# FanmingL/Recurrent-Offpolicy-RL

Hardware: AMD Instinct MI355X
Metric: env-steps/sec trained (higher is better)
Workload: dtype f32; 1 GPU; smamba_s32_c16_b2_nln SAC-REDQ update, B=64/GPU, T=1024, D=256 (configs[1]; N=8: configs[3]); row_length=1043, obs=17, act=6, critic=efc-8, global_rows=64, parallelism=dp1

## Files before the change

include/resel_hip.h:

```cpp
#ifndef RESEL_HIP_H
#define RESEL_HIP_H

#include <stddef.h>
#include <stdint.h>

#ifdef __cplusplus
extern "C" {
#endif

#define RESEL_OK 0
#define RESEL_EINVAL (-1)
#define RESEL_ELAUNCH (-2)

typedef void* resel_stream_t;

int resel_abi_version(void);
const char* resel_build_info(void);

enum {
    RESEL_PROF_SSCAN_FWD = 0, RESEL_PROF_SSCAN_BWD = 1, RESEL_PROF_ATTN_FWD = 2, RESEL_PROF_ATTN_DQ = 3, RESEL_PROF_ATTN_DKV = 4,
    RESEL_PROF_LINREC_REAL_FWD = 5, RESEL_PROF_LINREC_REAL_BWD = 6, RESEL_PROF_LINREC_COMPLEX_FWD = 7, RESEL_PROF_LINREC_COMPLEX_BWD = 8,
    RESEL_PROF_GRU_FWD = 9, RESEL_PROF_GRU_BWD = 10, RESEL_PROF_CONV_FWD = 11, RESEL_PROF_CONV_BWD = 12, RESEL_PROF_GEMM = 13,
    RESEL_PROF_SSCAN_FWD_LOCAL = 14, RESEL_PROF_SSCAN_BWD_LOCAL = 15,
    RESEL_PROF_NSLOTS = 16
// ... 123 lines not shown
                     const float* seg_lr, const float* seg_wd, int nseg, float beta1, float beta2, float eps,
                     int step, const float* grad_scale, resel_stream_t stream);
int resel_adamw_flat_bc(float* p, const float* g, float* m, float* v, int64_t n, const int64_t* seg_end,
                        const float* seg_lr, const float* seg_wd, int nseg, float beta1, float beta2, float eps,
                        float bc1, float bc2_sqrt, const float* grad_scale, resel_stream_t stream);
int resel_adamw_flat_dev(float* p, const float* g, float* m, float* v, int64_t n, const int64_t* seg_end,
                         const float* seg_lr, const float* seg_wd, int nseg, float beta1, float beta2, float eps,
                         const float* bias_corrections, const float* grad_scale, resel_stream_t stream);
size_t resel_sumsq_workspace_bytes(int64_t n);
int resel_sumsq(const float* x, int64_t n, float* out, void* workspace, resel_stream_t stream);

int resel_bias_act_fwd(float* y, const float* bias, int64_t rows, int C, int64_t rows_per_seg, int act, resel_stream_t stream);
size_t resel_bias_act_bwd_workspace_bytes(int64_t rows, int C, int64_t rows_per_seg);
int resel_bias_act_bwd(const float* g, int64_t ldg, const float* a, int64_t lda, float* gy, float* dbias, void* workspace, int64_t rows, int C,
                       int64_t rows_per_seg, int act, void* amax_gy, unsigned amax_epoch, resel_stream_t stream);

int resel_ensemble_head_fwd(float* y, const float* b2, const float* w3, const float* b3, float* q, int64_t rows, int H,
                            int64_t rows_per_seg, resel_stream_t stream);
size_t resel_ensemble_head_bwd_workspace_bytes(int64_t rows, int H, int64_t rows_per_seg);
int resel_ensemble_head_bwd(const float* gq, const float* a, const float* w3, float* gy, float* db2, float* dw3, void* workspace,
                            int64_t rows, int H, int64_t rows_per_seg, void* amax_gy, unsigned amax_epoch, resel_stream_t stream);

size_t resel_gemm_f32_workspace_bytes(int M, int N, int K, int batch);
int resel_gemm_f32(const float* A, int64_t lda, int64_t strideA, int a_kcontig,
                   const float* B, int64_t ldb, int64_t strideB, int b_kcontig,
                   const float* bias, int64_t strideBias, int act,
                   float* C, int64_t ldc, int64_t strideC, void* workspace,
                   int M, int N, int K, int batch, int split, resel_stream_t stream);

int resel_gemm_f32x(const float* A, int64_t lda, int64_t strideA, int a_kcontig,
// ... 4 lines not shown
                    void* amax_c, unsigned amax_epoch, resel_stream_t stream);
int resel_gemm_f32_fused_supported(int kind, int M, int N, int K, int64_t lda, int64_t ldb);
size_t resel_gemm_f32_fused_workspace_bytes(int M, int N, int K, int batch, int kind);
int resel_gemm_f32_dact(const float* A, int64_t lda, int64_t strideA, int a_kcontig,
                        const float* B, int64_t ldb, int64_t strideB, int b_kcontig,
                        const float* Y, int64_t ldy, int64_t strideY,
                        float* C, int64_t ldc, int64_t strideC, float* dbias, void* workspace,
                        int M, int N, int K, int batch, const float* amax_a, const float* amax_b,
                        void* amax_c, unsigned amax_epoch, resel_stream_t stream);
int resel_gemm_f32_head(const float* A, int64_t lda, int64_t strideA, int a_kcontig,
                        const float* B, int64_t ldb, int64_t strideB, int b_kcontig,
                        const float* bias, int64_t strideBias, const float* w3, int64_t strideW3, const float* b3,
                        float* C, int64_t ldc, int64_t strideC, float* q, void* workspace,
                        int M, int N, int K, int batch, const float* amax_a, const float* amax_b,
                        void* amax_c, unsigned amax_epoch, resel_stream_t stream);
int resel_place_blocks(float* out, int64_t ld_out, int rows, int cols, int nblk, const float* const* src, const int64_t* ld_src,
                       const int* r0, const int* nr, const int* c0, const int* nc, resel_stream_t stream);

int resel_amax_segments(const float* flat, const int64_t* begin, const int64_t* len, int nseg, void* handles, unsigned epoch,
                        resel_stream_t stream);
size_t resel_amax_state_bytes(void);
int resel_amax(const float* x, int64_t ld, int64_t stride, int rows, int cols, int batch, void* out, unsigned epoch, void* state,
               resel_stream_t stream);
int resel_amax_check(const float* x, int64_t ld, int64_t stride, int rows, int cols, int batch, const void* handle, int* err, int tag,
                     resel_stream_t stream);

size_t resel_gemm_bf16_workspace_bytes(int M, int N, int K);
int resel_gemm_bf16(const void* A, int64_t lda, int a_kcontig, int a_bf16, const void* B, int64_t ldb, int b_kcontig, int b_bf16,
                    const float* bias, void* C, int64_t ldc, int c_bf16, void* workspace, int M, int N, int K,
                    resel_stream_t stream);
// ... 28 lines not shown
```

recurrent-offpolicy-rl_amd/csrc/bias_act.hip:

```cpp
#include "resel_common.h"

namespace {
using namespace resel;

constexpr int BWD_ROWS = 128;

__device__ __forceinline__ float elu_(float x) { return x > 0.f ? x : fast_exp(x) - 1.f; }

__global__ __launch_bounds__(256) void bias_act_fwd_kernel(float* __restrict__ y, const float* __restrict__ bias, int64_t rows,
                                                           int C, int64_t rows_per_seg, int act) {
    const int c4n = C / 4;
    const int64_t n4 = rows * c4n;
    for (int64_t i = (int64_t)blockIdx.x * blockDim.x + threadIdx.x; i < n4; i += (int64_t)gridDim.x * blockDim.x) {
        const int64_t r = i / c4n;
        const int c = (int)(i % c4n) * 4;
        float4 v = ld4(y + r * C + c);
        if (bias) {
            const float4 b = ld4(bias + (r / rows_per_seg) * C + c);
            v.x += b.x; v.y += b.y; v.z += b.z; v.w += b.w;
        }
        if (act == 1) { v.x = elu_(v.x); v.y = elu_(v.y); v.z = elu_(v.z); v.w = elu_(v.w); }
        st4(y + r * C + c, v);
    }
}
// ... 87 lines not shown
    amax_publish_wave(gmax, amax);
    st4(&s_red[0][rl][cl * 4], accb);
    st4(&s_red[1][rl][cl * 4], accw);
    __syncthreads();
    if (rl < 2 && c < H) {
        float4 t = ld4(&s_red[rl][0][cl * 4]);
#pragma unroll
        for (int k = 1; k < 4; ++k) {
            const float4 qv = ld4(&s_red[rl][k][cl * 4]);
            t.x += qv.x; t.y += qv.y; t.z += qv.z; t.w += qv.w;
        }
        st4((rl == 0 ? db_part : dw_part) + ((seg * nrb + blockIdx.x) * (int64_t)H) + c, t);
    }
}

inline int row_blocks(int64_t rows_per_seg) { return (int)((rows_per_seg + BWD_ROWS - 1) / BWD_ROWS); }
inline int block_rows(int64_t, int, int64_t) { return BWD_ROWS; }
inline int row_blocks_of(int64_t rows_per_seg, int brows) { return (int)((rows_per_seg + brows - 1) / brows); }
inline bool shape_ok(int64_t rows, int C, int64_t rows_per_seg) {
    return rows > 0 && C > 0 && C % 4 == 0 && rows_per_seg > 0 && rows % rows_per_seg == 0;
}

}

extern "C" int resel_bias_act_fwd(float* y, const float* bias, int64_t rows, int C, int64_t rows_per_seg, int act,
                                  resel_stream_t stream) {
    if (!y || !shape_ok(rows, C, rows_per_seg) || act < 0 || act > 1 || !aligned16(y) || (bias && !aligned16(bias))) return RESEL_EINVAL;
    const int64_t n4 = rows * (C / 4);
    const int64_t want = (n4 + 255) / 256;
    const unsigned grid = (unsigned)(want < 256 * 32 ? want : 256 * 32);
// ... 39 lines not shown
                                       void* workspace, int64_t rows, int H, int64_t rows_per_seg, void* amax_gy, unsigned amax_epoch,
                                       resel_stream_t stream) {
    if (amax_gy && (reinterpret_cast<uintptr_t>(amax_gy) & 7u)) return RESEL_EINVAL;
    if (!gq || !a || !w3 || !gy || !db2 || !dw3 || !workspace || !shape_ok(rows, H, rows_per_seg)) return RESEL_EINVAL;
    if (!aligned16(a) || !aligned16(w3) || !aligned16(gy) || !aligned16(workspace)) return RESEL_EINVAL;
    const int nseg = (int)(rows / rows_per_seg), nrb = row_blocks(rows_per_seg);
    hipStream_t s = (hipStream_t)stream;
    float* db_part = (float*)workspace;
    float* dw_part = db_part + (size_t)nseg * nrb * H;
    hipLaunchKernelGGL(head_bwd_kernel, dim3(nrb, (H + 255) / 256, nseg), dim3(256), 0, s, gq, a, w3, gy, db_part, dw_part, H, rows_per_seg, nrb,
                       AmaxOut{(unsigned long long*)amax_gy, amax_epoch});
    launch_colsum(db_part, H, nrb, H, db2, s, 1, 0, nseg);
    launch_colsum(dw_part, H, nrb, H, dw3, s, 1, 0, nseg);
    return launch_status();
}
```

recurrent-offpolicy-rl_amd/csrc/gemm_bf3.hip:

```cpp
#include "gemm_splitk.h"
#include <type_traits>

namespace {
using namespace resel;

typedef float f32x16 __attribute__((ext_vector_type(16)));
typedef __bf16 bf16x8 __attribute__((ext_vector_type(8)));
constexpr int BM = 256, BN = 128;
constexpr int NTH = 512;
constexpr int GRID = 256;
constexpr int TILE = BM * BN;
constexpr int ROWB = 64;
constexpr int PLA = BM * ROWB, PLB = BN * ROWB;
constexpr int STAGE = 3 * PLA + 3 * PLB;

struct Params {
    const float *A, *B, *bias;
    float *C, *slab;
    int64_t lda, ldb, ldc, sA, sB, sC, sBias;
    int M, N, K;
    int act;
    int mt, nt;
    int nfull, nsplit, nsl, kslice;
    const float *amaxA, *amaxB;
// ... 882 lines not shown
#pragma unroll
                        for (int e = 0; e < 16; ++e) {
                            const int dm = (e & 3) + 8 * (e >> 2);
                            if (mb + dm < p.M) crow[(int64_t)dm * p.ldc] = v[e];
                        }
                    }
                    if (p.amaxC.slot) {
#pragma unroll
                        for (int e = 0; e < 16; e += 2) cmax = fmaxf(cmax, fmaxf(__builtin_fabsf(v[e]), __builtin_fabsf(v[e + 1])));
                    }
                }
            }
        } else {
            float* C = p.C + (int64_t)cur.z * p.sC;
            const bool full_m = cur.m0 + BM <= p.M;
            constexpr bool DACT = EPI == 4, HEAD = EPI == 5;
            const int act = EPI ? (HEAD ? 1 : 0) : p.act;
            if constexpr (DACT) {
                constexpr int PF = 3;
                const int lane = (int)__builtin_amdgcn_mbcnt_hi(~0u, __builtin_amdgcn_mbcnt_lo(~0u, 0u));
                const int li = lane & 31, lh = lane >> 5;
                const int w = __builtin_amdgcn_readfirstlane(threadIdx.x >> 6);
                const int wm = (w >> 1) * 128, wn = (w & 1) * 64;
                typedef float f32x4a __attribute__((ext_vector_type(4)));
                f32x4a yv[8][4];
                char* sc = lds + (w >> 1) * STAGE + 2 * PLA + (w & 1) * 5120;
                float* wr = reinterpret_cast<float*>(sc) + (4 * lh) * 40 + li;
                float4* rdp = reinterpret_cast<float4*>(sc + (lane >> 3) * 160 + (lane & 7) * 16);
                const uint32_t ylane = (uint32_t)(((lane >> 3) * (int)p.ldaux + 4 * (lane & 7)) * 4);
                const float* ybase = p.aux + (int64_t)cur.z * p.sAux + (int64_t)(cur.m0 + wm) * p.ldaux + cur.n0 + wn;
                auto yld = [](f32x4a& r, uint32_t off, const float* base) {
// ... 61 lines not shown
                char* sc = lds + (w >> 1) * STAGE + 2 * PLA + (w & 1) * 5120;
                float* wr = reinterpret_cast<float*>(sc) + (4 * lh) * 40 + li;
                const float4* rdp = reinterpret_cast<const float4*>(sc + (lane >> 3) * 160 + (lane & 7) * 16);
                auto tile = [&](int a, int b, const float4 (&yv)[4], float4& cs, const float4& w3, float (&qr)[4]) {
                    float v[16];
#pragma unroll
                    for (int e = 0; e < 16; ++e) v[e] = acc[a][b][e] + bv[b];
                    if (act == 1) {
#pragma unroll
                        for (int e = 0; e < 16; ++e) v[e] = elu1(v[e]);
                    }
                    if (act == 3) {
#pragma unroll
                        for (int e = 0; e < 16; ++e) v[e] = softplus_nb(v[e]);
                    }
                    if (p.amaxC.slot && !DACT) {
#pragma unroll
                        for (int e = 0; e < 16; e += 2) cmax = fmaxf(cmax, fmaxf(__builtin_fabsf(v[e]), __builtin_fabsf(v[e + 1])));
                    }
#pragma unroll
                    for (int e = 0; e < 16; ++e) wr[((e & 3) + 8 * (e >> 2)) * 40] = v[e];
                    float* q = C + (int64_t)(cur.m0 + wm + 32 * a + (lane >> 3)) * p.ldc + cur.n0 + wn + 32 * b + 4 * (lane & 7);
#pragma unroll
                    for (int g = 0; g < 4; ++g) {
                        float4 t = rdp[g * 8 * 10];
                        if (DACT) {
                            t.x *= yv[g].x > 0.f ? 1.f : yv[g].x + 1.f; t.y *= yv[g].y > 0.f ? 1.f : yv[g].y + 1.f;
                            t.z *= yv[g].z > 0.f ? 1.f : yv[g].z + 1.f; t.w *= yv[g].w > 0.f ? 1.f : yv[g].w + 1.f;
                            cs.x += t.x; cs.y += t.y; cs.z += t.z; cs.w += t.w;
                            if (p.amaxC.slot) cmax = amax4(cmax, t);
                        }
                        if (HEAD) qr[g] += (t.x * w3.x + t.y * w3.y) + (t.z * w3.z + t.w * w3.w);
                        if (p.ntst) {
                            typedef float f4v __attribute__((ext_vector_type(4)));
                            __builtin_nontemporal_store(f4v{t.x, t.y, t.z, t.w}, reinterpret_cast<f4v*>(q + (int64_t)(8 * g) * p.ldc));
                        } else {
                            *reinterpret_cast<float4*>(q + (int64_t)(8 * g) * p.ldc) = t;
                        }
                    }
                };
                if constexpr (EPI == 0) {
                    const float4 z4 = make_float4(0.f, 0.f, 0.f, 0.f);
                    const float4 nov[4] = {z4, z4, z4, z4};
                    float4 ncs = z4;
                    float nq[4] = {0.f, 0.f, 0.f, 0.f};
#pragma unroll
                    for (int b = 0; b < 2; ++b)
// ... 50 lines not shown
                    if (DACT) {
                        const float* yrow = p.aux + (int64_t)cur.z * p.sAux + (int64_t)mb * p.ldaux + n;
#pragma unroll
                        for (int e = 0; e < 16; ++e) {
                            const int dm = (e & 3) + 8 * (e >> 2);
                            float y = 0.f;
                            if (mb + dm < p.M) y = yrow[(int64_t)dm * p.ldaux]; else v[e] = 0.f;
                            v[e] *= y > 0.f ? 1.f : y + 1.f;
                            cs1[b] += v[e];
                        }
                    }
                    if (HEAD) {
                        const float w3 = p.aux[(int64_t)cur.z * p.sAux + n];
#pragma unroll
                        for (int e = 0; e < 16; ++e) qe[e] += v[e] * w3;
                    }
                    float* crow = C + (int64_t)mb * p.ldc + n;
                    if (act == 2) {
#pragma unroll
                        for (int e = 0; e < 16; ++e) {
                            const int dm = (e & 3) + 8 * (e >> 2);
                            if (mb + dm < p.M) v[e] += crow[(int64_t)dm * p.ldc];
                        }
                    }
                    if (full_m) {
#pragma unroll
                        for (int e = 0; e < 16; ++e) crow[(int64_t)((e & 3) + 8 * (e >> 2)) * p.ldc] = v[e];
                    } else {
#pragma unroll
                        for (int e = 0; e < 16; ++e) {
// ... 79 lines not shown
    Params p{A, B, bias, C, (float*)workspace, lda, ldb, ldc, strideA, strideB, strideC, strideBias, M, N, K, act,
             (M + BM - 1) / BM, (N + BN - 1) / BN, pl.nfull, pl.nsplit, pl.nsl, pl.kslice, amaxA, amaxB, AmaxOut{amax_c, amax_epoch}, g_nt,
             aux, ldaux, strideAux, red, redrows};
    const int64_t total = (int64_t)pl.nfull + (int64_t)pl.nsplit * pl.nsl;
    dim3 grid((unsigned)std::min<int64_t>(total, GRID));
    int rc;
#define BF3_LAUNCH(SP) \
    do { if (a_kcontig && b_kcontig) rc = launch_one<true, true, SP>(p, grid, s); \
         else if (a_kcontig) rc = launch_one<true, false, SP>(p, grid, s); \
         else if (b_kcontig) rc = launch_one<false, true, SP>(p, grid, s); \
         else rc = launch_one<false, false, SP>(p, grid, s); } while (0)
    const bool ws = split == 2 && K % BK == 0 && pl.kslice % BK == 0 && lda < (1 << 22) && ldb < (1 << 22);
    if (act >= 4) {
        if (!a_kcontig) return RESEL_EINVAL;
        if (act == 4) rc = b_kcontig ? launch_ws<true, true, 4>(p, grid, s) : launch_ws<true, false, 4>(p, grid, s);
        else rc = b_kcontig ? launch_ws<true, true, 5>(p, grid, s) : launch_ws<true, false, 5>(p, grid, s);
    } else if (ws) {
        if (a_kcontig && b_kcontig) rc = launch_ws<true, true>(p, grid, s);
        else if (a_kcontig) rc = launch_ws<true, false>(p, grid, s);
        else if (b_kcontig) rc = launch_ws<false, true>(p, grid, s);
        else rc = launch_ws<false, false>(p, grid, s);
    } else if (split == 3) BF3_LAUNCH(3); else if (split == 2) BF3_LAUNCH(2); else BF3_LAUNCH(6);
#undef BF3_LAUNCH
    if (rc != RESEL_OK) return rc;
    if (pl.nsplit) hipLaunchKernelGGL((gemm_fixup_kernel<BM, BN, Params>), dim3(TILE / 4 / 64, pl.nsplit), dim3(64, 4), 0, s, p);
#ifdef BF3_AB_FIXUP2
    if (pl.nsplit && act != 2) hipLaunchKernelGGL((gemm_fixup_kernel<BM, BN, Params>), dim3(TILE / 4 / 64, pl.nsplit), dim3(64, 4), 0, s, p);
#endif
    return launch_status();
}

// ... 2 lines not shown
```

recurrent-offpolicy-rl_amd/csrc/gemm_f32.hip:

```cpp
#include "gemm_splitk.h"

namespace resel {
size_t gemm_bf3_workspace_bytes(int M, int N, int K, int batch);
int gemm_bf3_launch(const float* A, int64_t lda, int64_t strideA, int a_kcontig, const float* B, int64_t ldb, int64_t strideB, int b_kcontig,
                    const float* bias, int64_t strideBias, int act, float* C, int64_t ldc, int64_t strideC, void* workspace,
                    int M, int N, int K, int batch, int split, hipStream_t s, const float* amaxA, const float* amaxB,
                    unsigned long long* amax_c, unsigned amax_epoch, const float* aux = nullptr, int64_t ldaux = 0, int64_t strideAux = 0,
                    float* red = nullptr, int redrows = 0);
bool gemm_bf3_fused_ok(int M, int N, int K, int64_t lda, int64_t ldb);
}

namespace {
using namespace resel;

typedef float f32x16 __attribute__((ext_vector_type(16)));
constexpr int BM = 128, BN = 128, NG = BK / 8;
constexpr int LDK = BK + 4;
constexpr int GRID = 512;
constexpr int TILE = BM * BN;

struct GemmParams {
    const float *A, *B, *bias;
    float *C, *slab;
    int64_t lda, ldb, ldc, sA, sB, sC, sBias;
// ... 542 lines not shown
    int rc = gemm_bf3_launch(A, lda, strideA, a_kcontig, B, ldb, strideB, b_kcontig, nullptr, 0, 4, C, ldc, strideC, nullptr, Mm, N, K, batch, 2,
                             s, amax_a, amax_b, (unsigned long long*)amax_c, amax_epoch, Y, ldy, strideY, part, rows);
    if (rc != RESEL_OK) return rc;
    if (tail) {
        char* ws2 = (char*)workspace + ((size_t)rows * N * batch * sizeof(float) + 255) / 256 * 256;
        rc = resel_gemm_f32x(A + (int64_t)Mm * lda, lda, strideA, 1, B, ldb, strideB, b_kcontig, nullptr, 0, 0, C + (int64_t)Mm * ldc, ldc, strideC, ws2,
                             tail, N, K, batch, 2, amax_a, amax_b, nullptr, 0u, stream);
        if (rc != RESEL_OK) return rc;
        hipLaunchKernelGGL(dact_tail_kernel, dim3((N + 63) / 64, batch), dim3(256), 0, s, C + (int64_t)Mm * ldc, ldc, strideC, Y + (int64_t)Mm * ldy, ldy, strideY,
                           tail, N, part ? part + (int64_t)(rows - 1) * N : nullptr, (int64_t)rows * N, AmaxOut{(unsigned long long*)amax_c, amax_epoch});
    }
    if (dbias) launch_colsum(part, N, rows, N, dbias, s, 1, 0, batch);
    return launch_status();
}

extern "C" int resel_gemm_f32_head(const float* A, int64_t lda, int64_t strideA, int a_kcontig,
                                   const float* B, int64_t ldb, int64_t strideB, int b_kcontig,
                                   const float* bias, int64_t strideBias, const float* w3, int64_t strideW3, const float* b3,
                                   float* C, int64_t ldc, int64_t strideC, float* q, void* workspace,
                                   int M, int N, int K, int batch, const float* amax_a, const float* amax_b,
                                   void* amax_c, unsigned amax_epoch, resel_stream_t stream) {
    if (!fused_args_ok(A, lda, strideA, a_kcontig, B, ldb, strideB, b_kcontig, C, ldc, M, N, K, batch, amax_a, amax_b, amax_c, workspace)) return RESEL_EINVAL;
    if (!w3 || !q || strideW3 % 4 || !aligned16(w3)) return RESEL_EINVAL;
    const int rc = gemm_bf3_launch(A, lda, strideA, a_kcontig, B, ldb, strideB, b_kcontig, bias, strideBias, 5, C, ldc, strideC, nullptr, M, N, K, batch, 2,
                                   (hipStream_t)stream, amax_a, amax_b, (unsigned long long*)amax_c, amax_epoch, w3, 0, strideW3, (float*)workspace);
    if (rc != RESEL_OK) return rc;
    hipLaunchKernelGGL(head_fold_kernel, dim3((M + 255) / 256, batch), dim3(256), 0, (hipStream_t)stream, (const float*)workspace,
                       2 * ((N + 127) / 128), M, b3, q);
    return launch_status();
}
```

recurrent-offpolicy-rl_amd/csrc/losses.hip:

```cpp
#include "resel_common.h"
#include <algorithm>

namespace {
using namespace resel;
constexpr int LOSS_BLOCKS = 256;

__device__ __forceinline__ void block_sum2(float a, float b, float* out2) {
    __shared__ float s[2][4];
    a = wave_sum(a); b = wave_sum(b);
    const int w = threadIdx.x >> 6;
    if ((threadIdx.x & 63) == 0) { s[0][w] = a; s[1][w] = b; }
    __syncthreads();
    if (threadIdx.x == 0) {
        out2[0] = (s[0][0] + s[0][1]) + (s[0][2] + s[0][3]);
        out2[1] = (s[1][0] + s[1][1]) + (s[1][2] + s[1][3]);
    }
}

__global__ __launch_bounds__(256) void q_loss_fwd_kernel(const float* __restrict__ q, const float* __restrict__ y, const float* __restrict__ mask,
                                                         float* __restrict__ part, int E, int M) {
    float acc = 0.f;
    for (int m = blockIdx.x * 256 + threadIdx.x; m < M; m += gridDim.x * 256) {
        const float mk = mask ? mask[m] : 1.f, t = y[m];
        float s = 0.f;
// ... 27 lines not shown
    block_sum2(acc, sl, part + 2 * blockIdx.x);
}
__global__ __launch_bounds__(256) void actor_loss_bwd_kernel(const float* __restrict__ q, const float* __restrict__ mask, const float* __restrict__ log_alpha,
                                                             const float* __restrict__ g, float* __restrict__ dlogp, float* __restrict__ dq, int E, int M,
                                                             int use_logp, int reduce_min) {
    const float gg = g[0], alpha = use_logp ? expf(log_alpha[0]) : 0.f;
    for (int m = blockIdx.x * 256 + threadIdx.x; m < M; m += gridDim.x * 256) {
        const float c = gg * (mask ? mask[m] : 1.f);
        if (dlogp) dlogp[m] = alpha * c;
        if (reduce_min) {
            int am = 0;
            float r = q[m];
            for (int e = 1; e < E; ++e) { const float v = q[(int64_t)e * M + m]; if (v < r) { r = v; am = e; } }
            for (int e = 0; e < E; ++e) dq[(int64_t)e * M + m] = e == am ? -c : 0.f;
        } else {
            const float v = -c / (float)E;
            for (int e = 0; e < E; ++e) dq[(int64_t)e * M + m] = v;
        }
    }
}
__global__ __launch_bounds__(256) void loss_final_kernel(const float* __restrict__ part, int nblk, float* __restrict__ out2) {
    float a = 0.f, b = 0.f;
    for (int i = threadIdx.x; i < nblk; i += 256) { a += part[2 * i]; b += part[2 * i + 1]; }
    block_sum2(a, b, out2);
}
inline int nblocks(int M) { return std::min(LOSS_BLOCKS, (M + 255) / 256); }
}

extern "C" size_t resel_masked_loss_workspace_bytes(void) { return (size_t)2 * LOSS_BLOCKS * sizeof(float); }

extern "C" int resel_q_loss_fwd(const float* q, const float* y, const float* mask, float* out2, void* workspace, int E, int M, resel_stream_t stream) {
    if (!q || !y || !out2 || !workspace || E <= 0 || M <= 0) return RESEL_EINVAL;
// ... 28 lines not shown
```

recurrent-offpolicy-rl_amd/csrc/misc.hip:

```cpp
#include "resel_common.h"
#include <cstdint>

extern "C" int resel_abi_version(void) { return 9; }

namespace { const unsigned long long* g_drop_base = nullptr; }
namespace resel { const unsigned long long* dropout_offset_base() { return g_drop_base; } }
extern "C" int resel_dropout_offset_base(const void* base) {
    if (base && ((uintptr_t)base & 7)) return RESEL_EINVAL;
    g_drop_base = (const unsigned long long*)base;
    return RESEL_OK;
}
extern "C" const char* resel_build_info(void) { return "resel_hip gfx950 (CDNA4, wave64) built " __DATE__ " " __TIME__; }

#include <utility>
#include <vector>
namespace resel {
namespace {
bool g_prof_enabled = false;
std::vector<std::pair<hipEvent_t, hipEvent_t>> g_prof_ev[RESEL_PROF_NSLOTS];
}
bool prof_on() { return g_prof_enabled; }
void prof_push(int slot, hipEvent_t a, hipEvent_t b) {
    if (slot >= 0 && slot < RESEL_PROF_NSLOTS) g_prof_ev[slot].emplace_back(a, b);
}
// ... 59 lines not shown
```

recurrent-offpolicy-rl_amd/offpolicy_rnn/hip/_lib.py:

```python
import ctypes
import os
from ctypes import c_float, c_int, c_int64, c_size_t, c_uint64, c_void_p

_HERE = os.path.dirname(os.path.abspath(__file__))
LIB_PATH = os.environ.get('RESEL_HIP_LIBRARY') or os.path.join(_HERE, 'libresel_hip.so')
ABI_VERSION = 9
_lib = None

P, I, L, F, S, U = c_void_p, c_int, c_int64, c_float, c_void_p, c_uint64
E = ctypes.c_uint

SIGNATURES = {
    'resel_abi_version': (c_int, []),
    'resel_build_info': (ctypes.c_char_p, []),
    'resel_profile_enable': (c_int, [I]),
    'resel_profile_collect': (c_int, [I, P, P]),
    'resel_selective_scan_ckpt_bytes': (c_size_t, [I, I, I, I]),
    'resel_selective_scan_fwd_workspace_bytes': (c_size_t, [I, I, I, I, I]),
    'resel_selective_scan_fwd': (c_int, [P, L, P, L, P, L, P, P, L, P, L, P, P, P, P, L, P, P, P, I, I, I, I, I, I, P, E, S]),
    'resel_selective_scan_bwd_workspace_bytes': (c_size_t, [I, I, I, I, I]),
    'resel_selective_scan_bwd': (c_int, [P, L, P, L, P, L, P, P, L, P, L, P, P, P, P, L, P,
                                         P, L, P, L, P, L, P, L, P, L, P, P, P, P, I, I, I, I, I, I, P, P, E, S]),
    'resel_causal_conv1d_fwd': (c_int, [P, L, P, P, P, P, L, I, I, I, I, I, P, E, S]),
    'resel_causal_conv1d_bwd_workspace_bytes': (c_size_t, [I, I, I, I]),
# ... 33 lines not shown
    'resel_q_loss_bwd': (c_int, [P, P, P, P, P, I, I, S]),
    'resel_actor_loss_fwd': (c_int, [P, P, P, P, P, P, I, I, I, I, S]),
    'resel_actor_loss_bwd': (c_int, [P, P, P, P, P, P, I, I, I, I, S]),
    'resel_sac_target_local': (c_int, [P, P, I, P, P, P, P, P, F, P, P, P, P, P, I, I, S]),
    'resel_guard_apply_slots': (c_int, [P, I, P, S]),
    'resel_sac_target_workspace_bytes': (c_size_t, [I]),
    'resel_soft_update': (c_int, [P, P, F, L, S]),
    'resel_adamw_flat': (c_int, [P, P, P, P, L, P, P, P, I, F, F, F, I, P, S]),
    'resel_adamw_flat_bc': (c_int, [P, P, P, P, L, P, P, P, I, F, F, F, F, F, P, S]),
    'resel_adamw_flat_dev': (c_int, [P, P, P, P, L, P, P, P, I, F, F, F, P, P, S]),
    'resel_sumsq_workspace_bytes': (c_size_t, [L]),
    'resel_sumsq': (c_int, [P, L, P, P, S]),
    'resel_bias_act_fwd': (c_int, [P, P, L, I, L, I, S]),
    'resel_bias_act_bwd_workspace_bytes': (c_size_t, [L, I, L]),
    'resel_bias_act_bwd': (c_int, [P, L, P, L, P, P, P, L, I, L, I, P, E, S]),
    'resel_ensemble_head_fwd': (c_int, [P, P, P, P, P, L, I, L, S]),
    'resel_ensemble_head_bwd_workspace_bytes': (c_size_t, [L, I, L]),
    'resel_ensemble_head_bwd': (c_int, [P, P, P, P, P, P, P, L, I, L, P, E, S]),
    'resel_gemm_f32_workspace_bytes': (c_size_t, [I, I, I, I]),
    'resel_gemm_f32': (c_int, [P, L, L, I, P, L, L, I, P, L, I, P, L, L, P, I, I, I, I, I, S]),
    'resel_gemm_f32x': (c_int, [P, L, L, I, P, L, L, I, P, L, I, P, L, L, P, I, I, I, I, I, P, P, P, E, S]),
    'resel_amax_segments': (c_int, [P, P, P, I, P, E, S]),
    'resel_amax_state_bytes': (c_size_t, []),
    'resel_amax': (c_int, [P, L, L, I, I, I, P, E, P, S]),
    'resel_gemm_f32_fused_supported': (c_int, [I, I, I, I, L, L]),
    'resel_gemm_f32_fused_workspace_bytes': (c_size_t, [I, I, I, I, I]),
    'resel_gemm_f32_dact': (c_int, [P, L, L, I, P, L, L, I, P, L, L, P, L, L, P, P, I, I, I, I, P, P, P, E, S]),
    'resel_gemm_f32_head': (c_int, [P, L, L, I, P, L, L, I, P, L, P, L, P, P, L, L, P, P, I, I, I, I, P, P, P, E, S]),
    'resel_amax_check': (c_int, [P, L, L, I, I, I, P, P, I, S]),
    'resel_gemm_bf16_workspace_bytes': (c_size_t, [I, I, I]),
    'resel_gemm_bf16': (c_int, [P, L, I, I, P, L, I, I, P, P, L, I, P, I, I, I, S]),
    'resel_colsum_bf16_workspace_bytes': (c_size_t, [I, I]),
    'resel_colsum_bf16': (c_int, [P, L, I, I, P, P, S]),
    'resel_gather_trajs': (c_int, [P, I, L, P, I, I, I, I, I, I, I, I, I, P, I, P, S]),
    'resel_mamba_conv_step': (c_int, [P, L, P, L, P, L, L, L, I, P, P, P, I, I, I, I, S]),
    'resel_selective_state_update': (c_int, [P, L, P, L, P, P, L, P, P, P, P, P, L, P, I, I, I, I, S]),
    'resel_atb_workspace_bytes': (c_size_t, [L, I, I]),
    'resel_atb': (c_int, [P, L, I, P, L, I, P, I, P, L, S]),
    'resel_attn_decode': (c_int, [P, L, P, P, I, P, P, F, I, I, I, I, S]),
}


class ReselHipUnavailable(RuntimeError):
# ... 29 lines not shown
```

recurrent-offpolicy-rl_amd/offpolicy_rnn/hip/ops.py:

```python
import ctypes
import os
from typing import Optional

import torch

from ._lib import check, lib


def _need_cuda(name, *ts):
    for t in ts:
        if t is not None and not t.is_cuda:
            raise RuntimeError(f'RESeL-HIP: {name} needs CUDA tensors (got a {t.device} tensor); the HIP kernels are the '
                               f'only implementation of this op - there is no CPU fallback.')


def _p(t: Optional[torch.Tensor]):
    return None if t is None else ctypes.c_void_p(t.data_ptr())


if hasattr(torch._C, '_cuda_getCurrentRawStream') and hasattr(torch._C, '_cuda_getDevice'):
    def _stream():
        return ctypes.c_void_p(torch._C._cuda_getCurrentRawStream(torch._C._cuda_getDevice()))
else:
    def _stream():
# ... 855 lines not shown
        la = log_alpha.detach().float().reshape(-1).contiguous()
        out = torch.empty(2, dtype=torch.float32, device=q.device)
        ws = _ws(lib().resel_masked_loss_workspace_bytes(), q.device)
        check(lib().resel_actor_loss_fwd(_p(lp), _p(q2), _p(m1), _p(la), _p(out), _p(ws), E, M, int(bool(use_logp)), int(bool(reduce_min)), _stream()),
              'actor_loss_fwd')
        ctx.save_for_backward(q2, m1, la)
        ctx.cfg = (bool(use_logp), bool(reduce_min), q.shape, None if logp is None else logp.shape)
        return out

    @staticmethod
    def backward(ctx, g2):
        q2, m1, la = ctx.saved_tensors
        g = g2[0:1]
        use_logp, reduce_min, qshape, lshape = ctx.cfg
        E, M = q2.shape
        dq = torch.empty_like(q2)
        dlp = torch.empty(M, dtype=torch.float32, device=q2.device) if use_logp else None
        check(lib().resel_actor_loss_bwd(_p(q2), _p(m1), _p(la), _p(g.float().reshape(1).contiguous()), _p(dlp), _p(dq), E, M, int(use_logp),
                                         int(reduce_min), _stream()), 'actor_loss_bwd')
        return (None if dlp is None or lshape is None else dlp.view(lshape)), dq.view(qshape), None, None, None, None


def masked_actor_loss(logp, q, mask, log_alpha, use_logp=True, reduce_min=False):
    out = MaskedActorLossFn.apply(logp, q, mask, log_alpha, use_logp, reduce_min)
    return out[0], out[1].detach()


@torch.no_grad()
def guard_apply_slots(slots, world, guard):
    _need_cuda('guard_apply_slots', slots, guard)
    check(lib().resel_guard_apply_slots(_p(slots), int(world), _p(guard), _stream()), 'guard_apply_slots')


ACT_IDS = {None: 0, 'linear': 0, 'elu': 1}
# ... 18 lines not shown
    rows, C = g2.shape
    aid = ACT_IDS[act]
    if aid == 0 and not need_dbias:
        return g2, None
    if aid and not (a2.dim() == 2 and a2.stride(1) == 1 and a2.stride(0) >= C and a2.stride(0) % 4 == 0 and a2.data_ptr() % 16 == 0):
        a2 = a2.contiguous()
    gy = torch.empty(rows, C, dtype=torch.float32, device=g2.device) if aid else g2
    nseg = rows // int(rows_per_seg)
    db = torch.empty(nseg, C, dtype=torch.float32, device=g2.device) if need_dbias else None
    ws = _ws(lib().resel_bias_act_bwd_workspace_bytes(rows, C, int(rows_per_seg)), g2.device) if need_dbias else None
    slot, slot_p, epoch = _slot_args(amax_tracking() and rows * C >= (1 << 20), g2.device)
    check(lib().resel_bias_act_bwd(_p(g2), g2.stride(0), _p(a2) if aid else None, a2.stride(0) if aid else 0, _p(gy) if aid else None, _p(db), _p(ws), rows, C, int(rows_per_seg), aid,
                                   slot_p, epoch, _stream()), 'bias_act_bwd')
    tag_amax(gy, slot)
    return gy, db


@torch.no_grad()
def ensemble_head_fwd_(y3, b2, w3, b3):
    _need_cuda('ensemble_head', y3, b2, w3, b3)
    E, M, H = y3.shape
    q = torch.empty(E, M, dtype=torch.float32, device=y3.device)
    check(lib().resel_ensemble_head_fwd(_p(y3), _p(b2), _p(w3), _p(b3), _p(q), E * M, H, M, _stream()), 'ensemble_head_fwd')
    tag_amax(y3, None)
    return q


@torch.no_grad()
def ensemble_head_bwd(gq, a3, w3):
    _need_cuda('ensemble_head_bwd', gq, a3, w3)
# ... 594 lines not shown
    if AMAX_VERIFY:
        _verify_operands(A, B, ha, hb, f'gemm_dact M={M} N={N} K={K} batch={batch}')
    GEMM_FLOPS[0] += 2.0 * M * N * K * batch
    L = lib()
    ws = _ws(L.resel_gemm_f32_fused_workspace_bytes(M, N, K, batch, 4), A.device)
    dbias = torch.empty(batch, N, dtype=torch.float32, device=A.device) if need_dbias else None
    multi = batched and batch > 1
    slot, slot_p, epoch = _slot_args(amax_tracking() and M * N * batch >= (1 << 20), A.device)
    check(L.resel_gemm_f32_dact(_p(A), A.stride(-2), A.stride(0) if multi else 0, 1, _p(B), B.stride(-2), B.stride(0) if multi else 0, int(b_kcontig),
                                _p(Y), Y.stride(-2), Y.stride(0) if multi else 0, _p(out), out.stride(-2), out.stride(0) if multi else 0,
                                _p(dbias), _p(ws), M, N, K, batch, _p(ha), _p(hb), slot_p, epoch, _stream()), 'gemm_f32_dact')
    return _gemm_done(out, slot, 2), dbias


@torch.no_grad()
def gemm_f32_head(A, B, b_kcontig, bias, w3, b3, amax_a=None, amax_b=None):
    _need_cuda('gemm_f32_head', A, B, bias, w3)
    batch, M, K = A.shape
    N = B.shape[-2] if b_kcontig else B.shape[-1]
    assert A.stride(-1) == 1 and B.stride(-1) == 1 and w3.shape == (batch, N) and w3.is_contiguous() and bias.shape == (batch, N) and bias.stride(-1) == 1
    ha, hb = _forced_handles(A, B, amax_a, amax_b)
    if AMAX_VERIFY:
        _verify_operands(A, B, ha, hb, f'gemm_head M={M} N={N} K={K} batch={batch}')
    GEMM_FLOPS[0] += 2.0 * M * N * K * batch
    L = lib()
    ws = _ws(L.resel_gemm_f32_fused_workspace_bytes(M, N, K, batch, 5), A.device)
    a = torch.empty(batch, M, N, dtype=torch.float32, device=A.device)
    q = torch.empty(batch, M, dtype=torch.float32, device=A.device)
    multi = batch > 1
    slot, slot_p, epoch = _slot_args(amax_tracking() and M * N * batch >= (1 << 20), A.device)
    check(L.resel_gemm_f32_head(_p(A), A.stride(-2), A.stride(0) if multi else 0, 1, _p(B), B.stride(-2), B.stride(0) if multi else 0, int(b_kcontig),
                                _p(bias), bias.stride(0) if multi else 0, _p(w3), N, _p(b3), _p(a), a.stride(-2), a.stride(0) if multi else 0, _p(q), _p(ws),
                                M, N, K, batch, _p(ha), _p(hb), slot_p, epoch, _stream()), 'gemm_f32_head')
    return _gemm_done(a, slot, 2), q


@torch.no_grad()
def conv_step(x, window, weight, bias, d_conv, layout, act):
    _need_cuda('conv_step', x, window)
    B, Di, K = x.shape[0], x.shape[1], d_conv
    W, sd, sk = (K, K, 1) if layout == 'dk' else (K - 1, 1, Di)
    assert window.shape == (B, Di * W) and window.stride(1) == 1 and x.stride(1) == 1
    new = torch.empty((B, Di * W), dtype=torch.float32, device=x.device)
    xc = torch.empty((B, Di), dtype=torch.float32, device=x.device)
    check(lib().resel_mamba_conv_step(_p(x), x.stride(0), _p(window), window.stride(0), _p(new), new.stride(0), sd, sk, W,
                                      _p(weight), _p(bias), _p(xc), B, Di, K, int(bool(act)), _stream()), 'mamba_conv_step')
# ... 77 lines not shown
```

recurrent-offpolicy-rl_amd/offpolicy_rnn/models/ensemble_linear_model.py:

```python
import torch
import torch.nn as nn

from ..hip import ops


def _unit(t):
    return t if t.stride(-1) == 1 else t.contiguous()


class _SharedInput(torch.autograd.Function):

    @staticmethod
    def forward(ctx, x2, weight, bias, act, x_part=None, col0=0, ax=None):
        E, n_in, n_out = weight.shape
        w_cat = weight.permute(1, 0, 2).reshape(n_in, E * n_out)
        x2 = x2 if x2.stride(-1) == 1 else x2.contiguous()
        y2 = ops.gemm_f32(x2, w_cat, True, False, None if bias is None else bias.reshape(E * n_out), act, amax_a=ax,
                          amax_b=ops.weight_amax(weight))
        ax = ax if ax is not None else ops.amax_of(x2)
        ctx.save_for_backward(x2, w_cat, y2 if act is not None else None)
        ctx.ax = ops.keep_handles(ax)[0]
        ctx.dims = (E, n_in, n_out, bias is not None, act)
        ctx.part = None if x_part is None else (col0, x_part.shape[-1], tuple(x_part.shape))
        return y2.view(-1, E, n_out).transpose(0, 1)
# ... 96 lines not shown


class _CriticMLP(torch.autograd.Function):

    @staticmethod
    def forward(ctx, x2, W1, b1, W2, b2, W3, b3, x_part, col0, ax):
        E, n_in, H1 = W1.shape
        H2 = W2.shape[2]
        M = x2.shape[0]
        w_cat = W1.permute(1, 0, 2).reshape(n_in, E * H1)
        y2 = ops.gemm_f32(x2, w_cat, True, False, b1.reshape(E * H1), 'elu', amax_a=ax, amax_b=ops.weight_amax(W1))
        h_x = ax if ax is not None else ops.amax_of(x2)
        h_a1 = ops.amax_of(y2)
        a1 = y2.view(M, E, H1).transpose(0, 1)
        w3v = W3.reshape(E, H2)
        a2, q = ops.gemm_f32_head(a1, W2, False, b2.reshape(E, H2), w3v, None if b3 is None else b3.reshape(E), amax_a=h_a1,
                                  amax_b=ops.weight_amax(W2))
        ctx.save_for_backward(x2, w_cat, y2, W2, w3v, a2)
        ctx.handles = ops.keep_handles(h_x, h_a1)
        ctx.dims = (E, n_in, H1, H2, M, b3 is not None)
        ctx.part = None if x_part is None else (col0, x_part.shape[-1], tuple(x_part.shape))
        return q.view(E, M, 1)

    @staticmethod
    def backward(ctx, gq):
        x2, w_cat, y2, W2, w3v, a2 = ctx.saved_tensors
        E, n_in, H1, H2, M, has_b3 = ctx.dims
        h_x, h_a1 = ops.live_handles(ctx.handles)
        need = ctx.needs_input_grad
        gq2 = gq.reshape(E, M)
        gy2, db2, dw3 = ops.ensemble_head_bwd(gq2, a2, w3v)
        a1 = y2.view(M, E, H1).transpose(0, 1)
        dw2 = _member_wgrad(a1, gy2, h_a1) if need[3] else None
        db3 = gq2.sum(dim=1).view(E, 1, 1) if (has_b3 and need[6]) else None
        g1 = torch.empty(M, E, H1, dtype=torch.float32, device=x2.device).transpose(0, 1)
        _, db1 = ops.gemm_f32_dact(gy2, W2, True, a1, g1, need_dbias=bool(need[2]), amax_b=ops.weight_amax(W2))
        g2 = g1.transpose(0, 1).reshape(M, E * H1)
        ops.tag_amax(g2, ops.amax_of(g1))
        dx = ops.gemm_f32(g2, w_cat, True, True) if need[0] else None
        dw1 = None
        if need[1]:
            dw1 = ops.gemm_f32(x2, g2, False, False, amax_a=h_x).view(n_in, E, H1).permute(1, 0, 2)
        dpart = None
        if ctx.part is not None and need[7]:
            col0, k, shape = ctx.part
            dpart = ops.gemm_f32(g2, w_cat[col0:col0 + k], True, True).view(shape)
        return (dx, dw1, None if db1 is None else db1.view(E, 1, H1), dw2, db2.view(E, 1, H2) if need[4] else None,
                dw3.view(E, H2, 1) if need[5] else None, db3, dpart, None, None)


def critic_mlp_fusable(l0, act0, l1, act1, l2, act2, x) -> bool:
    if not (isinstance(l0, EnsembleLinear) and isinstance(l1, EnsembleLinear) and isinstance(l2, EnsembleLinear)):
        return False
    elu = lambda a: isinstance(a, nn.ELU) and a.alpha == 1.0
    if not (elu(act0) and elu(act1) and isinstance(act2, nn.Identity) and l0.use_bias and l1.use_bias):
        return False
    E = l0.active_members()
    if l1.active_members() != E or l2.active_members() != E or x.dtype != torch.float32 or not x.is_cuda:
        return False
    n_in, H1 = l0.weight.shape[1:]
    H2 = l1.weight.shape[2]
    if l1.weight.shape[1] != H1 or l2.weight.shape[1] != H2 or l2.weight.shape[2] != 1 or x.shape[-1] != n_in:
        return False
    nd = x.dim()
# ... 86 lines not shown
```

Baseline: 3.230 million env-steps/s.

## Fuse frozen-critic head derivative into forward GEMM for actor-loss backward

When the critic is evaluated for the actor loss with frozen weights, the forward head GEMM now also stores w3 times the ELU derivative instead of the activation. Backward then skips ensemble_head_bwd and the weight gradients. When dq is uniform across members, the per-row scale is applied after the input-gradient GEMMs rather than before. The actor loss backward also writes a single dq row that is broadcast by expand. This removes a head-backward kernel and writes to E-wide buffers, at the cost of a new epilogue variant and an extra row_scale pass on small outputs.

```diff
diff --git a/include/resel_hip.h b/include/resel_hip.h
--- a/include/resel_hip.h
+++ b/include/resel_hip.h
@@ -161,6 +161,9 @@
 size_t resel_bias_act_bwd_workspace_bytes(int64_t rows, int C, int64_t rows_per_seg);
 int resel_bias_act_bwd(const float* g, int64_t ldg, const float* a, int64_t lda, float* gy, float* dbias, void* workspace, int64_t rows, int C,
                        int64_t rows_per_seg, int act, void* amax_gy, unsigned amax_epoch, resel_stream_t stream);
+
+int resel_row_scale(const float* x, int64_t ldx, int64_t strideX, const float* r, int64_t strideR, float* out, int64_t ldo, int64_t strideO,
+                    int64_t rows, int C, int batch, void* amax_out, unsigned amax_epoch, resel_stream_t stream);
 
 int resel_ensemble_head_fwd(float* y, const float* b2, const float* w3, const float* b3, float* q, int64_t rows, int H,
                             int64_t rows_per_seg, resel_stream_t stream);
@@ -195,6 +198,12 @@
                         float* C, int64_t ldc, int64_t strideC, float* q, void* workspace,
                         int M, int N, int K, int batch, const float* amax_a, const float* amax_b,
                         void* amax_c, unsigned amax_epoch, resel_stream_t stream);
+int resel_gemm_f32_head_dq(const float* A, int64_t lda, int64_t strideA, int a_kcontig,
+                           const float* B, int64_t ldb, int64_t strideB, int b_kcontig,
+                           const float* bias, int64_t strideBias, const float* w3, int64_t strideW3, const float* b3,
+                           float* C, int64_t ldc, int64_t strideC, float* q, void* workspace,
+                           int M, int N, int K, int batch, const float* amax_a, const float* amax_b,
+                           void* amax_c, unsigned amax_epoch, resel_stream_t stream);
 int resel_place_blocks(float* out, int64_t ld_out, int rows, int cols, int nblk, const float* const* src, const int64_t* ld_src,
                        const int* r0, const int* nr, const int* c0, const int* nc, resel_stream_t stream);
 
diff --git a/recurrent-offpolicy-rl_amd/csrc/bias_act.hip b/recurrent-offpolicy-rl_amd/csrc/bias_act.hip
--- a/recurrent-offpolicy-rl_amd/csrc/bias_act.hip
+++ b/recurrent-offpolicy-rl_amd/csrc/bias_act.hip
@@ -125,6 +125,23 @@
     }
 }
 
+__global__ __launch_bounds__(256) void row_scale_kernel(const float* x, int64_t ldx, int64_t sx, const float* __restrict__ r, int64_t sr,
+                                                        float* out, int64_t ldo, int64_t so, int64_t rows, int C, int64_t n4, AmaxOut amax) {
+    const int c4n = C / 4;
+    float mx = 0.f;
+    for (int64_t i = (int64_t)blockIdx.x * blockDim.x + threadIdx.x; i < n4; i += (int64_t)gridDim.x * blockDim.x) {
+        const int64_t row = i / c4n;
+        const int c = (int)(i - row * c4n) * 4;
+        const int64_t b = row / rows, m = row - b * rows;
+        const float s = r[b * sr + m];
+        float4 v = ld4(x + b * sx + m * ldx + c);
+        v.x *= s; v.y *= s; v.z *= s; v.w *= s;
+        st4(out + b * so + m * ldo + c, v);
+        mx = amax4(mx, v);
+    }
+    amax_publish_wave(mx, amax);
+}
+
 inline int row_blocks(int64_t rows_per_seg) { return (int)((rows_per_seg + BWD_ROWS - 1) / BWD_ROWS); }
 inline int block_rows(int64_t, int, int64_t) { return BWD_ROWS; }
 inline int row_blocks_of(int64_t rows_per_seg, int brows) { return (int)((rows_per_seg + brows - 1) / brows); }
@@ -194,3 +211,17 @@
     launch_colsum(dw_part, H, nrb, H, dw3, s, 1, 0, nseg);
     return launch_status();
 }
+
+extern "C" int resel_row_scale(const float* x, int64_t ldx, int64_t strideX, const float* r, int64_t strideR, float* out, int64_t ldo, int64_t strideO,
+                               int64_t rows, int C, int batch, void* amax_out, unsigned amax_epoch, resel_stream_t stream) {
+    if (amax_out && (reinterpret_cast<uintptr_t>(amax_out) & 7u)) return RESEL_EINVAL;
+    if (!x || !r || !out || rows <= 0 || C <= 0 || C % 4 || batch <= 0 || ldx < C || ldo < C || (ldx & 3) || (ldo & 3)) return RESEL_EINVAL;
+    if (batch > 1 && ((strideX & 3) || (strideO & 3) || strideX < 0 || strideO < 0 || strideR < 0)) return RESEL_EINVAL;
+    if (!aligned16(x) || !aligned16(out)) return RESEL_EINVAL;
+    const int64_t n4 = (int64_t)batch * rows * (C / 4);
+    const int64_t want = (n4 + 255) / 256;
+    const unsigned grid = (unsigned)(want < 256 * 32 ? want : 256 * 32);
+    hipLaunchKernelGGL(row_scale_kernel, dim3(grid), dim3(256), 0, (hipStream_t)stream, x, ldx, strideX, r, strideR, out, ldo, strideO, rows, C, n4,
+                       AmaxOut{(unsigned long long*)amax_out, amax_epoch});
+    return launch_status();
+}
diff --git a/recurrent-offpolicy-rl_amd/csrc/gemm_bf3.hip b/recurrent-offpolicy-rl_amd/csrc/gemm_bf3.hip
--- a/recurrent-offpolicy-rl_amd/csrc/gemm_bf3.hip
+++ b/recurrent-offpolicy-rl_amd/csrc/gemm_bf3.hip
@@ -920,7 +920,8 @@
         } else {
             float* C = p.C + (int64_t)cur.z * p.sC;
             const bool full_m = cur.m0 + BM <= p.M;
-            constexpr bool DACT = EPI == 4, HEAD = EPI == 5;
+            constexpr bool DACT = EPI == 4, HEAD = EPI == 5 || EPI == 6;
+            constexpr bool DQ = EPI == 6;
             const int act = EPI ? (HEAD ? 1 : 0) : p.act;
             if constexpr (DACT) {
                 constexpr int PF = 3;
@@ -1012,7 +1013,7 @@
 #pragma unroll
                         for (int e = 0; e < 16; ++e) v[e] = softplus_nb(v[e]);
                     }
-                    if (p.amaxC.slot && !DACT) {
+                    if (p.amaxC.slot && !DACT && !DQ) {
 #pragma unroll
                         for (int e = 0; e < 16; e += 2) cmax = fmaxf(cmax, fmaxf(__builtin_fabsf(v[e]), __builtin_fabsf(v[e + 1])));
                     }
@@ -1029,6 +1030,11 @@
                             if (p.amaxC.slot) cmax = amax4(cmax, t);
                         }
                         if (HEAD) qr[g] += (t.x * w3.x + t.y * w3.y) + (t.z * w3.z + t.w * w3.w);
+                        if constexpr (DQ) {
+                            t.x = w3.x * (t.x > 0.f ? 1.f : t.x + 1.f); t.y = w3.y * (t.y > 0.f ? 1.f : t.y + 1.f);
+                            t.z = w3.z * (t.z > 0.f ? 1.f : t.z + 1.f); t.w = w3.w * (t.w > 0.f ? 1.f : t.w + 1.f);
+                            if (p.amaxC.slot) cmax = amax4(cmax, t);
+                        }
                         if (p.ntst) {
                             typedef float f4v __attribute__((ext_vector_type(4)));
                             __builtin_nontemporal_store(f4v{t.x, t.y, t.z, t.w}, reinterpret_cast<f4v*>(q + (int64_t)(8 * g) * p.ldc));
@@ -1109,6 +1115,10 @@
                         const float w3 = p.aux[(int64_t)cur.z * p.sAux + n];
 #pragma unroll
                         for (int e = 0; e < 16; ++e) qe[e] += v[e] * w3;
+                        if constexpr (DQ) {
+#pragma unroll
+                            for (int e = 0; e < 16; ++e) v[e] = w3 * (v[e] > 0.f ? 1.f : v[e] + 1.f);
+                        }
                     }
                     float* crow = C + (int64_t)mb * p.ldc + n;
                     if (act == 2) {
@@ -1218,7 +1228,9 @@
     if (act >= 4) {
         if (!a_kcontig) return RESEL_EINVAL;
         if (act == 4) rc = b_kcontig ? launch_ws<true, true, 4>(p, grid, s) : launch_ws<true, false, 4>(p, grid, s);
-        else rc = b_kcontig ? launch_ws<true, true, 5>(p, grid, s) : launch_ws<true, false, 5>(p, grid, s);
+        else if (act == 5) rc = b_kcontig ? launch_ws<true, true, 5>(p, grid, s) : launch_ws<true, false, 5>(p, grid, s);
+        else if (act == 6) rc = b_kcontig ? launch_ws<true, true, 6>(p, grid, s) : launch_ws<true, false, 6>(p, grid, s);
+        else return RESEL_EINVAL;
     } else if (ws) {
         if (a_kcontig && b_kcontig) rc = launch_ws<true, true>(p, grid, s);
         else if (a_kcontig) rc = launch_ws<true, false>(p, grid, s);
diff --git a/recurrent-offpolicy-rl_amd/csrc/gemm_f32.hip b/recurrent-offpolicy-rl_amd/csrc/gemm_f32.hip
--- a/recurrent-offpolicy-rl_amd/csrc/gemm_f32.hip
+++ b/recurrent-offpolicy-rl_amd/csrc/gemm_f32.hip
@@ -580,18 +580,38 @@
     return launch_status();
 }
 
+namespace {
+int head_entry(int epi, const float* A, int64_t lda, int64_t strideA, int a_kcontig, const float* B, int64_t ldb, int64_t strideB, int b_kcontig,
+               const float* bias, int64_t strideBias, const float* w3, int64_t strideW3, const float* b3, float* C, int64_t ldc, int64_t strideC,
+               float* q, void* workspace, int M, int N, int K, int batch, const float* amax_a, const float* amax_b, void* amax_c, unsigned amax_epoch,
+               resel_stream_t stream) {
+    if (!fused_args_ok(A, lda, strideA, a_kcontig, B, ldb, strideB, b_kcontig, C, ldc, M, N, K, batch, amax_a, amax_b, amax_c, workspace)) return RESEL_EINVAL;
+    if (!w3 || !q || strideW3 % 4 || !aligned16(w3)) return RESEL_EINVAL;
+    const int rc = gemm_bf3_launch(A, lda, strideA, a_kcontig, B, ldb, strideB, b_kcontig, bias, strideBias, epi, C, ldc, strideC, nullptr, M, N, K, batch, 2,
+                                   (hipStream_t)stream, amax_a, amax_b, (unsigned long long*)amax_c, amax_epoch, w3, 0, strideW3, (float*)workspace);
+    if (rc != RESEL_OK) return rc;
+    hipLaunchKernelGGL(head_fold_kernel, dim3((M + 255) / 256, batch), dim3(256), 0, (hipStream_t)stream, (const float*)workspace,
+                       2 * ((N + 127) / 128), M, b3, q);
+    return launch_status();
+}
+}
+
 extern "C" int resel_gemm_f32_head(const float* A, int64_t lda, int64_t strideA, int a_kcontig,
                                    const float* B, int64_t ldb, int64_t strideB, int b_kcontig,
                                    const float* bias, int64_t strideBias, const float* w3, int64_t strideW3, const float* b3,
                                    float* C, int64_t ldc, int64_t strideC, float* q, void* workspace,
                                    int M, int N, int K, int batch, const float* amax_a, const float* amax_b,
                                    void* amax_c, unsigned amax_epoch, resel_stream_t stream) {
-    if (!fused_args_ok(A, lda, strideA, a_kcontig, B, ldb, strideB, b_kcontig, C, ldc, M, N, K, batch, amax_a, amax_b, amax_c, workspace)) return RESEL_EINVAL;
-    if (!w3 || !q || strideW3 % 4 || !aligned16(w3)) return RESEL_EINVAL;
-    const int rc = gemm_bf3_launch(A, lda, strideA, a_kcontig, B, ldb, strideB, b_kcontig, bias, strideBias, 5, C, ldc, strideC, nullptr, M, N, K, batch, 2,
-                                   (hipStream_t)stream, amax_a, amax_b, (unsigned long long*)amax_c, amax_epoch, w3, 0, strideW3, (float*)workspace);
-    if (rc != RESEL_OK) return rc;
-    hipLaunchKernelGGL(head_fold_kernel, dim3((M + 255) / 256, batch), dim3(256), 0, (hipStream_t)stream, (const float*)workspace,
-                       2 * ((N + 127) / 128), M, b3, q);
-    return launch_status();
-}
+    return head_entry(5, A, lda, strideA, a_kcontig, B, ldb, strideB, b_kcontig, bias, strideBias, w3, strideW3, b3, C, ldc, strideC, q, workspace,
+                      M, N, K, batch, amax_a, amax_b, amax_c, amax_epoch, stream);
+}
+
+extern "C" int resel_gemm_f32_head_dq(const float* A, int64_t lda, int64_t strideA, int a_kcontig,
+                                      const float* B, int64_t ldb, int64_t strideB, int b_kcontig,
+                                      const float* bias, int64_t strideBias, const float* w3, int64_t strideW3, const float* b3,
+                                      float* C, int64_t ldc, int64_t strideC, float* q, void* workspace,
+                                      int M, int N, int K, int batch, const float* amax_a, const float* amax_b,
+                                      void* amax_c, unsigned amax_epoch, resel_stream_t stream) {
+    return head_entry(6, A, lda, strideA, a_kcontig, B, ldb, strideB, b_kcontig, bias, strideBias, w3, strideW3, b3, C, ldc, strideC, q, workspace,
+                      M, N, K, batch, amax_a, amax_b, amax_c, amax_epoch, stream);
+}
diff --git a/recurrent-offpolicy-rl_amd/csrc/losses.hip b/recurrent-offpolicy-rl_amd/csrc/losses.hip
--- a/recurrent-offpolicy-rl_amd/csrc/losses.hip
+++ b/recurrent-offpolicy-rl_amd/csrc/losses.hip
@@ -65,8 +65,7 @@
             for (int e = 1; e < E; ++e) { const float v = q[(int64_t)e * M + m]; if (v < r) { r = v; am = e; } }
             for (int e = 0; e < E; ++e) dq[(int64_t)e * M + m] = e == am ? -c : 0.f;
         } else {
-            const float v = -c / (float)E;
-            for (int e = 0; e < E; ++e) dq[(int64_t)e * M + m] = v;
+            dq[m] = -c / (float)E;
         }
     }
 }
diff --git a/recurrent-offpolicy-rl_amd/csrc/misc.hip b/recurrent-offpolicy-rl_amd/csrc/misc.hip
--- a/recurrent-offpolicy-rl_amd/csrc/misc.hip
+++ b/recurrent-offpolicy-rl_amd/csrc/misc.hip
@@ -1,7 +1,7 @@
 #include "resel_common.h"
 #include <cstdint>
 
-extern "C" int resel_abi_version(void) { return 9; }
+extern "C" int resel_abi_version(void) { return 10; }
 
 namespace { const unsigned long long* g_drop_base = nullptr; }
 namespace resel { const unsigned long long* dropout_offset_base() { return g_drop_base; } }
diff --git a/recurrent-offpolicy-rl_amd/offpolicy_rnn/hip/_lib.py b/recurrent-offpolicy-rl_amd/offpolicy_rnn/hip/_lib.py
--- a/recurrent-offpolicy-rl_amd/offpolicy_rnn/hip/_lib.py
+++ b/recurrent-offpolicy-rl_amd/offpolicy_rnn/hip/_lib.py
@@ -4,7 +4,7 @@
 
 _HERE = os.path.dirname(os.path.abspath(__file__))
 LIB_PATH = os.environ.get('RESEL_HIP_LIBRARY') or os.path.join(_HERE, 'libresel_hip.so')
-ABI_VERSION = 9
+ABI_VERSION = 10
 _lib = None
 
 P, I, L, F, S, U = c_void_p, c_int, c_int64, c_float, c_void_p, c_uint64
@@ -71,6 +71,7 @@
     'resel_bias_act_fwd': (c_int, [P, P, L, I, L, I, S]),
     'resel_bias_act_bwd_workspace_bytes': (c_size_t, [L, I, L]),
     'resel_bias_act_bwd': (c_int, [P, L, P, L, P, P, P, L, I, L, I, P, E, S]),
+    'resel_row_scale': (c_int, [P, L, L, P, L, P, L, L, L, I, I, P, E, S]),
     'resel_ensemble_head_fwd': (c_int, [P, P, P, P, P, L, I, L, S]),
     'resel_ensemble_head_bwd_workspace_bytes': (c_size_t, [L, I, L]),
     'resel_ensemble_head_bwd': (c_int, [P, P, P, P, P, P, P, L, I, L, P, E, S]),
@@ -84,6 +85,7 @@
     'resel_gemm_f32_fused_workspace_bytes': (c_size_t, [I, I, I, I, I]),
     'resel_gemm_f32_dact': (c_int, [P, L, L, I, P, L, L, I, P, L, L, P, L, L, P, P, I, I, I, I, P, P, P, E, S]),
     'resel_gemm_f32_head': (c_int, [P, L, L, I, P, L, L, I, P, L, P, L, P, P, L, L, P, P, I, I, I, I, P, P, P, E, S]),
+    'resel_gemm_f32_head_dq': (c_int, [P, L, L, I, P, L, L, I, P, L, P, L, P, P, L, L, P, P, I, I, I, I, P, P, P, E, S]),
     'resel_amax_check': (c_int, [P, L, L, I, I, I, P, P, I, S]),
     'resel_gemm_bf16_workspace_bytes': (c_size_t, [I, I, I]),
     'resel_gemm_bf16': (c_int, [P, L, I, I, P, L, I, I, P, P, L, I, P, I, I, I, S]),
diff --git a/recurrent-offpolicy-rl_amd/offpolicy_rnn/hip/ops.py b/recurrent-offpolicy-rl_amd/offpolicy_rnn/hip/ops.py
--- a/recurrent-offpolicy-rl_amd/offpolicy_rnn/hip/ops.py
+++ b/recurrent-offpolicy-rl_amd/offpolicy_rnn/hip/ops.py
@@ -893,10 +893,12 @@
         g = g2[0:1]
         use_logp, reduce_min, qshape, lshape = ctx.cfg
         E, M = q2.shape
-        dq = torch.empty_like(q2)
+        dq = torch.empty_like(q2) if reduce_min else torch.empty(M, dtype=torch.float32, device=q2.device)
         dlp = torch.empty(M, dtype=torch.float32, device=q2.device) if use_logp else None
         check(lib().resel_actor_loss_bwd(_p(q2), _p(m1), _p(la), _p(g.float().reshape(1).contiguous()), _p(dlp), _p(dq), E, M, int(use_logp),
                                          int(reduce_min), _stream()), 'actor_loss_bwd')
+        if not reduce_min:
+            dq = dq.view(1, M).expand(E, M)
         return (None if dlp is None or lshape is None else dlp.view(lshape)), dq.view(qshape), None, None, None, None
 
 
@@ -945,6 +947,29 @@
                                    slot_p, epoch, _stream()), 'bias_act_bwd')
     tag_amax(gy, slot)
     return gy, db
+
+
+@torch.no_grad()
+def row_scale(x, r, out=None):
+    _need_cuda('row_scale', x, r)
+    batched = x.dim() == 3
+    batch = x.shape[0] if batched else 1
+    M, C = x.shape[-2], x.shape[-1]
+    assert x.dtype == torch.float32 and r.dtype == torch.float32 and x.stride(-1) == 1 and tuple(r.shape) == tuple(x.shape[:-1])
+    if M > 1 and r.stride(-1) != 1:
+        r = r.contiguous()
+    if out is None:
+        out = torch.empty(tuple(x.shape), dtype=torch.float32, device=x.device)
+    assert out.shape == x.shape and out.stride(-1) == 1
+    multi = batched and batch > 1
+    slot, slot_p, epoch = _slot_args(amax_tracking() and batch * M * C >= (1 << 20), x.device)
+    check(lib().resel_row_scale(_p(x), x.stride(-2), x.stride(0) if multi else 0, _p(r), r.stride(0) if multi else 0, _p(out), out.stride(-2),
+                                out.stride(0) if multi else 0, M, C, batch, slot_p, epoch, _stream()), 'row_scale')
+    return tag_amax(out, slot)
+
+
+def actor_head_on():
+    return os.environ.get('RESEL_ACTOR_HEAD', '1') != '0'
 
 
 @torch.no_grad()
@@ -1569,7 +1594,7 @@
 
 
 @torch.no_grad()
-def gemm_f32_head(A, B, b_kcontig, bias, w3, b3, amax_a=None, amax_b=None):
+def gemm_f32_head(A, B, b_kcontig, bias, w3, b3, amax_a=None, amax_b=None, dq=False):
     _need_cuda('gemm_f32_head', A, B, bias, w3)
     batch, M, K = A.shape
     N = B.shape[-2] if b_kcontig else B.shape[-1]
@@ -1584,7 +1609,7 @@
     q = torch.empty(batch, M, dtype=torch.float32, device=A.device)
     multi = batch > 1
     slot, slot_p, epoch = _slot_args(amax_tracking() and M * N * batch >= (1 << 20), A.device)
-    check(L.resel_gemm_f32_head(_p(A), A.stride(-2), A.stride(0) if multi else 0, 1, _p(B), B.stride(-2), B.stride(0) if multi else 0, int(b_kcontig),
+    check((L.resel_gemm_f32_head_dq if dq else L.resel_gemm_f32_head)(_p(A), A.stride(-2), A.stride(0) if multi else 0, 1, _p(B), B.stride(-2), B.stride(0) if multi else 0, int(b_kcontig),
                                 _p(bias), bias.stride(0) if multi else 0, _p(w3), N, _p(b3), _p(a), a.stride(-2), a.stride(0) if multi else 0, _p(q), _p(ws),
                                 M, N, K, batch, _p(ha), _p(hb), slot_p, epoch, _stream()), 'gemm_f32_head')
     return _gemm_done(a, slot, 2), q
diff --git a/recurrent-offpolicy-rl_amd/offpolicy_rnn/models/ensemble_linear_model.py b/recurrent-offpolicy-rl_amd/offpolicy_rnn/models/ensemble_linear_model.py
--- a/recurrent-offpolicy-rl_amd/offpolicy_rnn/models/ensemble_linear_model.py
+++ b/recurrent-offpolicy-rl_amd/offpolicy_rnn/models/ensemble_linear_model.py
@@ -134,10 +134,13 @@
         h_a1 = ops.amax_of(y2)
         a1 = y2.view(M, E, H1).transpose(0, 1)
         w3v = W3.reshape(E, H2)
+        need = ctx.needs_input_grad
+        ctx.frozen = (ops.actor_head_on() and any(need) and not any(need[1:7]) and n_in % 4 == 0
+                      and (x_part is None or x_part.shape[-1] % 4 == 0))
         a2, q = ops.gemm_f32_head(a1, W2, False, b2.reshape(E, H2), w3v, None if b3 is None else b3.reshape(E), amax_a=h_a1,
-                                  amax_b=ops.weight_amax(W2))
+                                  amax_b=ops.weight_amax(W2), dq=ctx.frozen)
         ctx.save_for_backward(x2, w_cat, y2, W2, w3v, a2)
-        ctx.handles = ops.keep_handles(h_x, h_a1)
+        ctx.handles = ops.keep_handles(h_x, h_a1, ops.amax_of(a2))
         ctx.dims = (E, n_in, H1, H2, M, b3 is not None)
         ctx.part = None if x_part is None else (col0, x_part.shape[-1], tuple(x_part.shape))
         return q.view(E, M, 1)
@@ -146,9 +149,11 @@
     def backward(ctx, gq):
         x2, w_cat, y2, W2, w3v, a2 = ctx.saved_tensors
         E, n_in, H1, H2, M, has_b3 = ctx.dims
-        h_x, h_a1 = ops.live_handles(ctx.handles)
+        h_x, h_a1, h_a2 = ops.live_handles(ctx.handles)
         need = ctx.needs_input_grad
         gq2 = gq.reshape(E, M)
+        if ctx.frozen:
+            return _CriticMLP._backward_frozen(ctx, gq2, x2, w_cat, y2, W2, a2, h_a2)
         gy2, db2, dw3 = ops.ensemble_head_bwd(gq2, a2, w3v)
         a1 = y2.view(M, E, H1).transpose(0, 1)
         dw2 = _member_wgrad(a1, gy2, h_a1) if need[3] else None
@@ -168,6 +173,28 @@
         return (dx, dw1, None if db1 is None else db1.view(E, 1, H1), dw2, db2.view(E, 1, H2) if need[4] else None,
                 dw3.view(E, H2, 1) if need[5] else None, db3, dpart, None, None)
 
+    @staticmethod
+    def _backward_frozen(ctx, gq2, x2, w_cat, y2, W2, s2, h_s2):
+        E, n_in, H1, H2, M, _ = ctx.dims
+        need = ctx.needs_input_grad
+        a1 = y2.view(M, E, H1).transpose(0, 1)
+        uniform = E == 1 or gq2.stride(0) == 0
+        if uniform:
+            r, gy2 = gq2[0], s2
+        else:
+            r, gy2, h_s2 = None, ops.row_scale(s2, gq2), None
+        g1 = torch.empty(M, E, H1, dtype=torch.float32, device=x2.device).transpose(0, 1)
+        ops.gemm_f32_dact(gy2, W2, True, a1, g1, need_dbias=False, amax_a=h_s2, amax_b=ops.weight_amax(W2))
+        g2 = g1.transpose(0, 1).reshape(M, E * H1)
+        ops.tag_amax(g2, ops.amax_of(g1))
+        scale = (lambda t: ops.row_scale(t, r, out=t)) if uniform else (lambda t: t)
+        dx = scale(ops.gemm_f32(g2, w_cat, True, True)) if need[0] else None
+        dpart = None
+        if ctx.part is not None and need[7]:
+            col0, k, shape = ctx.part
+            dpart = scale(ops.gemm_f32(g2, w_cat[col0:col0 + k], True, True)).view(shape)
+        return dx, None, None, None, None, None, None, dpart, None, None
+
 
 def critic_mlp_fusable(l0, act0, l1, act1, l2, act2, x) -> bool:
     if not (isinstance(l0, EnsembleLinear) and isinstance(l1, EnsembleLinear) and isinstance(l2, EnsembleLinear)):
```

Measured after the change: 3.226 million env-steps/s, median of 2. About the same (-0.1%).
